# RuruX/femo

Measured on AMD Instinct MI355X. Metric: DOFs/sec assemble+adjoint-solve, 10M-DOF Poisson, 1/2/4/8 MI355X, higher is better.
Workload: dtype f64

## Files before the change

femo_amd/_lib.py:

```python
from __future__ import annotations

import ctypes as C
import os
from typing import Optional

_HERE = os.path.dirname(os.path.abspath(__file__))
LIB_PATH = os.environ.get("FEMO_LIB") or os.path.join(_HERE, "csrc", "libfemo_hip.so")

c_i64 = C.c_int64
c_i32p = C.POINTER(C.c_int32)
c_i64p = C.POINTER(C.c_int64)
c_f64p = C.POINTER(C.c_double)
H = C.c_void_p

ABI_VERSION = 10
MESH_INFO_COUNT = 12
MESH_INFO_KEYS = ("tdim", "n_vert", "n_rows", "n_cell", "nnz", "sell_entries", "max_rowlen",
                  "max_valence", "n_slices", "visit_entries", "regular_slices", "short_slices")

PDE_POISSON = 0
PDE_NL_POISSON = 1
PDE_MASS = 2
PDE_EB_BEAM = 3
J_L2_TRACKING = 0
# ... 89 lines not shown
    "femo_ctx_newton_flag_info": (C.c_int, [H, c_i64p, C.c_int]),
    "femo_mesh_create": (C.c_int, [H, C.c_int, c_i64, c_i64, C.c_void_p, c_i64, C.c_void_p, C.POINTER(H)]),
    "femo_mesh_destroy": (C.c_int, [H]),
    "femo_mesh_info": (C.c_int, [H, c_i64p]),
    "femo_mesh_set_boundary_facets": (C.c_int, [H, C.c_void_p]),
    "femo_pc_plan_host": (C.c_int, [C.c_int, C.c_int64, C.c_void_p, C.c_void_p, C.c_void_p, C.c_int64, C.POINTER(C.c_int32),
                          C.c_void_p, C.POINTER(C.c_int64), C.c_void_p, C.c_void_p, C.c_void_p, C.c_void_p, C.c_void_p]),
    "femo_emu_group_create": (C.c_int, [C.c_int, C.POINTER(H)]),
    "femo_emu_group_destroy": (C.c_int, [H]),
    "femo_comm_emulate": (C.c_int, [H, H, C.c_int]),
    "femo_comm_model": (C.c_int, [H, C.c_int, C.c_int]),
    "femo_comm_stats": (C.c_int, [H, C.POINTER(C.c_int64), C.c_int]),
    "femo_mesh_pcg_info": (C.c_int, [H, C.POINTER(C.c_int64), C.c_int]),
    "femo_mesh_head_info": (C.c_int, [H, C.POINTER(C.c_int64), C.c_int]),
    "femo_mesh_tail_info": (C.c_int, [H, C.POINTER(C.c_int64), C.c_int]),
    "femo_shell_create": (C.c_int, [H, c_i64, C.c_void_p, c_i64, C.c_void_p, c_i64, C.c_void_p, C.c_void_p, C.c_void_p, C.c_void_p, C.POINTER(H)]),
    "femo_shell_destroy": (C.c_int, [H]),
    "femo_shell_pc_create": (C.c_int, [H, C.c_int, c_i64, C.c_int, C.c_void_p] + [C.c_void_p] * 11),
    "femo_shell_pc_coarse": (C.c_int, [H, C.c_int, C.c_void_p, c_i64] + [C.c_void_p] * 6),
    "femo_shell_pc_coarse_matrix": (C.c_int, [H, H, C.c_void_p, C.c_int, C.c_void_p, C.POINTER(c_i64)]),
    "femo_shell_pc_hermite": (C.c_int, [H] + [C.c_void_p] * 11),
    "femo_shell_pc_info": (C.c_int, [H, C.POINTER(C.c_int32)]),
    "femo_shell_pc_block_items": (C.c_int, [H, C.c_int64] + [C.c_void_p] * 4),
    "femo_shell_pc_weights": (C.c_int, [H, C.c_double, C.c_double]),
    "femo_shell_pc_apply": (C.c_int, [H, H, C.c_void_p, H, H]),
    "femo_shell_pnorm_stress": (C.c_int, [H, C.c_double, C.c_double, H, H, C.c_double, C.c_double, C.c_double, C.c_double,
                                          C.POINTER(C.c_double), C.c_int, H, H]),
    "femo_shell_vm_rhs": (C.c_int, [H, C.c_double, C.c_double, H, H, C.c_double, H, H]),
    "femo_shell_p1_mass": (C.c_int, [H, H, H]),
    "femo_shell_ndof": (c_i64, [H]),
# ... 105 lines not shown
    "femo_elast_pc_setup": (C.c_int, [H, C.c_double]),
    "femo_elast_pc_info": (C.c_int, [H, c_i64p]),
    "femo_elast_pc_export_level": (C.c_int, [H, C.c_int, C.c_void_p]),
    "femo_elast_pc_apply": (C.c_int, [H, H, H]),
    "femo_elast_bench_spmv": (C.c_int, [H, H, H, C.c_int, c_f64p]),
    "femo_filter_create": (C.c_int, [H, C.c_int, c_i64, C.c_void_p, C.c_double, C.POINTER(H)]),
    "femo_filter_destroy": (C.c_int, [H]),
    "femo_filter_nnz": (C.c_int, [H, c_i64p]),
    "femo_filter_apply": (C.c_int, [H, C.c_int, H, H]),
    "femo_filter_export_csr": (C.c_int, [H, C.c_int, C.c_void_p, C.c_void_p, C.c_void_p]),
}


OPTIONAL = frozenset({"femo_mesh_pcg_info", "femo_mesh_head_info", "femo_mat_identity_solve_flag", "femo_vec_axpy_if",
                      "femo_newton_rhs_linear_if", "femo_ctx_newton_flag_info", "femo_mesh_tail_info",
                      "femo_dRdf_cell_apply_T_add_to_host", "femo_vec_get_host_promised", "femo_host_forget"})


class FemoError(RuntimeError):
    pass


_lib: Optional[C.CDLL] = None


def load() -> C.CDLL:
    global _lib
    if _lib is not None:
        return _lib
    if not os.path.exists(LIB_PATH):
        raise FemoError(
# ... 27 lines not shown
```

femo_amd/csrc/api.hip:

```cpp
#include <algorithm>

#include <atomic>

#include "femo_internal.h"

std::atomic<long long> femo_host_sync_count{0};

void femo_mat_touch(femo_mat* A) {
  static std::atomic<uint64_t> next{0};
  if (A) A->gen = ++next;
}

namespace {

__global__ void k_fill(int64_t n, double v, double* __restrict__ x) {
  for (int64_t i = (int64_t)blockIdx.x * blockDim.x + threadIdx.x; i < n; i += (int64_t)gridDim.x * blockDim.x) x[i] = v;
}

__global__ void k_axpy(int64_t n, double a, const double* __restrict__ x, double* __restrict__ y,
                       const int32_t* __restrict__ run_if, int32_t* __restrict__ count) {
  if (run_if != nullptr) {
    const bool leave = *run_if == 0;
    if (blockIdx.x == 0 && threadIdx.x == 0) atomicAdd(count + (leave ? 0 : 1), 1);
    if (leave) return;
// ... 523 lines not shown
  A->mesh = m;
  const int64_t nd = std::max<int64_t>(m->n_slices * FEMO_WAVE, 1);
  FEMO_HIP_CHECK(hipMalloc(&A->d_diag, nd * sizeof(double)));
  FEMO_HIP_CHECK(hipMalloc(&A->d_vals, std::max<int64_t>(m->sell_entries, 1) * sizeof(double) + 64));
  FEMO_HIP_CHECK(hipMemsetAsync(A->d_diag, 0, nd * sizeof(double), m->ctx->stream));
  FEMO_HIP_CHECK(hipMemsetAsync(A->d_vals, 0, std::max<int64_t>(m->sell_entries, 1) * sizeof(double), m->ctx->stream));
  *out = A;
  return 0;
}

int femo_mat_destroy(femo_mat* A) {
  if (!A) return 0;
  hipStreamSynchronize(A->mesh->ctx->stream);
  hipFree(A->d_diag); hipFree(A->d_vals); hipFree(A->d_valsT); hipFree(A->d_valsS); hipFree(A->d_s);
  hipFree(A->d_pcmask); hipFree(A->d_idrows);
  delete A;
  return 0;
}

static int note_pinned_vertices(femo_mat* A, int pde, const double* params, const femo_bc* bc) {
  femo_mesh* m = A->mesh;
  if (bc != nullptr && bc->n > 0) {
    if (A->idrows_uid != bc->uid) {
      const int64_t nb = std::max<int64_t>(m->n_vert, 1) + 64;
      if (!A->d_idrows) FEMO_HIP_CHECK(hipMalloc(&A->d_idrows, nb));
      FEMO_HIP_CHECK(hipMemcpyAsync(A->d_idrows, bc->d_mask, nb, hipMemcpyDeviceToDevice, m->ctx->stream));
      A->idrows_uid = bc->uid;
    }
    A->has_idrows = true;
  } else {
// ... 216 lines not shown
  if (m->n_rows == 0) return 0;
  int64_t* d_rp = nullptr; int32_t* d_col = nullptr; double* d_val = nullptr;
  FEMO_HIP_CHECK(hipMalloc(&d_rp, rp.size() * sizeof(int64_t)));
  FEMO_HIP_CHECK(hipMalloc(&d_col, m->nnz * sizeof(int32_t)));
  FEMO_HIP_CHECK(hipMalloc(&d_val, m->nnz * sizeof(double)));
  FEMO_HIP_CHECK(hipMemcpyAsync(d_rp, rp.data(), rp.size() * sizeof(int64_t), hipMemcpyHostToDevice, st));
  hipLaunchKernelGGL(k_export_rows, dim3((unsigned)((m->n_rows + 255) / 256)), dim3(256), 0, st, m->n_rows, m->d_mptr, m->d_cols, m->d_rowlen, m->d_rowreal, A->d_diag, A->d_vals, d_rp, d_col, d_val);
  FEMO_HIP_CHECK(hipGetLastError());
  FEMO_HIP_CHECK(hipMemcpyAsync(col, d_col, m->nnz * sizeof(int32_t), hipMemcpyDeviceToHost, st));
  FEMO_HIP_CHECK(hipMemcpyAsync(val, d_val, m->nnz * sizeof(double), hipMemcpyDeviceToHost, st));
  FEMO_HIP_CHECK(hipStreamSynchronize(st));
  hipFree(d_rp); hipFree(d_col); hipFree(d_val);
  return 0;
}

int femo_mat_diagonal(const femo_mat* A, femo_vec* d) {
  FEMO_REQUIRE(A && d, "null argument");
  FEMO_REQUIRE(d->n >= A->mesh->n_rows, "vector too small");
  femo_vec_touch(d);
  FEMO_HIP_CHECK(hipMemcpyAsync(d->d, A->d_diag, A->mesh->n_rows * sizeof(double), hipMemcpyDeviceToDevice, A->mesh->ctx->stream));
  return 0;
}

int femo_functional_value(femo_mesh* m, int kind, const double* params, const femo_vec* u,
                          const femo_vec* f, const femo_vec* u_d, double* value) {
  FEMO_REQUIRE(m && u && f && u_d && value, "null argument");
  FEMO_REQUIRE(u->n >= m->n_vert && u_d->n >= m->n_vert && f->n >= m->n_cell, "vector size mismatch in functional");
  if (m->n_nbr > 0) FEMO_TRY(femo_halo_exchange(m, const_cast<femo_vec*>(u)));
  const uint64_t key[4] = {u->uid, u->gen, u_d->uid, u_d->gen};
  return femo_launch_functional_value(m, kind, params, u->d, f->d, u_d->d, value, key);
// ... 142 lines not shown
```

femo_amd/csrc/femo_internal.h:

```cpp
#pragma once

#include <hip/hip_runtime.h>
#include <rccl/rccl.h>

#include <cstdint>
#include <cstdlib>
#include <cstdio>
#include <cstring>
#include <string>
#include <vector>

#include "femo_hip.h"
#include "femo_hip_test.h"

void femo_set_error(const char* fmt, ...);

#include <atomic>
extern std::atomic<long long> femo_host_sync_count;
inline hipError_t femo_counted_stream_sync(hipStream_t s) { femo_host_sync_count.fetch_add(1, std::memory_order_relaxed); return hipStreamSynchronize(s); }
inline hipError_t femo_counted_event_sync(hipEvent_t e) { femo_host_sync_count.fetch_add(1, std::memory_order_relaxed); return hipEventSynchronize(e); }
inline hipError_t femo_counted_device_sync() { femo_host_sync_count.fetch_add(1, std::memory_order_relaxed); return hipDeviceSynchronize(); }
#define hipStreamSynchronize(s) femo_counted_stream_sync(s)
#define hipEventSynchronize(e) femo_counted_event_sync(e)
#define hipDeviceSynchronize() femo_counted_device_sync()
// ... 303 lines not shown
  double* d_dense = nullptr;
  uint64_t* d_rowmask = nullptr;
  uint64_t uid = 0;
};

struct femo_mat {
  femo_mesh* mesh = nullptr;
  double* d_diag = nullptr;
  double* d_vals = nullptr;
  double* d_valsT = nullptr;
  bool valsT_valid = false;
  double* d_valsS = nullptr;
  double* d_s = nullptr;
  bool scaled_valid = false, scaled_transposed = false;
  bool s_valid = false;
  uint8_t* d_idrows = nullptr;
  bool has_idrows = false;
  uint64_t idrows_uid = 0;
  bool bpx_ok = false;
  uint8_t* d_pcmask = nullptr;
  bool pc_has_mask = false;
  uint64_t pc_key = 0;
  uint64_t gen = 0;
};
void femo_mat_touch(femo_mat* A);

#if defined(__HIPCC__)
__device__ __forceinline__ double femo_wave_sum(double v) {
#pragma unroll
  for (int off = 32; off > 0; off >>= 1) v += __shfl_down(v, off, 64);
// ... 83 lines not shown
  double* partials = nullptr;
  const double* dvec = nullptr;
  const int32_t* done = nullptr;
  const int32_t* slices = nullptr;
  int64_t n_slices = 0;
  hipStream_t stream = nullptr;
  bool ghost = false;
};
int femo_launch_spmv(const femo_mat* A, const double* x, double* y, const FemoSpmv& d);
int femo_halo_spmv(const femo_mat* A, double* x, double* y, const FemoSpmv& d, int* g_int, int* g_bnd, bool inflight = false);
int femo_halo_raw(femo_mesh* m, double* x, hipStream_t st);
int femo_spmv_transposed_scatter(const femo_mat* A, const double* vals, bool unit, const double* x, double* y, const int32_t* done);
inline bool femo_transpose_is_local(const femo_mesh* m) { return m->n_nbr == 0; }
int femo_mat_ensure_s(femo_mat* A);
int femo_mat_ensure_scaled(femo_mat* A, bool transpose);
int femo_launch_newton_rhs_linear(const femo_mat* K, const double* x, const double* u, const double* load,
                                  const uint8_t* bcmask, const double* bcval, double* y, int64_t slice0 = 0, int64_t n_range = -1,
                                  const int32_t* run_if = nullptr, int32_t* count = nullptr);
int femo_poisson_load_vector(femo_mesh* m, const femo_vec* f, const double** load);
int femo_poisson_load_stream_begin(femo_mesh* m, const femo_vec* f, int* n_ranges);
int femo_poisson_load_stream_range(femo_mesh* m, const femo_vec* f, int k, int64_t* slice0, int64_t* n_slices);
int femo_launch_impose_bc(femo_mesh* m, const double* u, const uint8_t* bcmask, const double* bcval, const double** ubc,
                          const int32_t* run_if = nullptr);
inline bool femo_residual_is_pipelined(const femo_mesh* m) {
  const int nbr = (m->max_rowlen + 1) & ~1;
  return nbr <= (m->tdim == 3 ? 16 : 8);
}
int femo_spmv_grid(const femo_mesh* m);
int femo_halo_exchange_on(femo_mesh* m, femo_vec* x, hipStream_t st);
int femo_mesh_classify_slices(femo_mesh* m);
// ... 73 lines not shown
```

femo_amd/csrc/solver.hip:

```cpp
#include <algorithm>
#include <climits>
#include <cmath>
#include <cstdlib>

#include "femo_internal.h"

namespace {

constexpr int S_GAMMA = 0, S_DELTA = 2, S_TOL2 = 3;
constexpr int P_DELTA = 0, P_GAMMA = 1;

__global__ __launch_bounds__(FEMO_BLOCK) void k_cg_init(int64_t n, const double* __restrict__ b, const double* __restrict__ q,
                                                        const double* __restrict__ s, double* __restrict__ r,
                                                        double* __restrict__ p, double* __restrict__ xh,
                                                        double* __restrict__ partials, const uint8_t* __restrict__ idrow) {
  __shared__ double lds[FEMO_BLOCK / 64];
  double s0 = 0.0, s1 = 0.0;
  for (int64_t i = (int64_t)blockIdx.x * FEMO_BLOCK + threadIdx.x; i < n; i += (int64_t)gridDim.x * FEMO_BLOCK) {
    const double si = s[i], bi = si * b[i];
    const double ri = q ? si * (b[i] - q[i]) : bi;
    if (idrow != nullptr && idrow[i]) {
      r[i] = 0.0; p[i] = 0.0; xh[i] = ri;
      continue;
    }
// ... 595 lines not shown
}

static int fill_info(femo_ctx* ctx, hipEvent_t end, femo_solve_info* info, int iters, int conv, double rr) {
  float ms = 0.f;
  FEMO_HIP_CHECK(hipEventElapsedTime(&ms, ctx->ev0, end));
  info->iterations = iters;
  info->converged = conv;
  info->residual_norm = std::sqrt(rr);
  info->solve_ms = ms;
  return 0;
}

static int finish_solve(femo_mat* A, const double* xh, femo_vec* x, bool zero_guess, femo_solve_info* info, int iters,
                        int conv, double rr) {
  FEMO_TRY(unscale_x(A, xh, x, zero_guess));
  return fill_info(A->mesh->ctx, A->mesh->ctx->ev1, info, iters, conv, rr);
}

struct SpmvSamples {
  static constexpr int N = 4;
  femo_ctx* ctx;
  int from;
  int n = 0;
  bool on = false;
  SpmvSamples(femo_ctx* c, int first) : ctx(c), from(first) {}
  int begin(int it) {
    on = it >= from && it < from + N;
    if (on) FEMO_HIP_CHECK(hipEventRecord(ctx->ev_pool[2 * n], ctx->stream));
    return 0;
  }
// ... 148 lines not shown
  V.x = w.xh; V.r = w.r; V.p = p0; V.q = nullptr; V.n = n; V.cur = 0; V.gv = gv; V.atol2 = 0.0;
  V.nb_q[0] = V.nb_q[1] = 0; V.Pq[0] = V.Pq[1] = nullptr;
  FEMO_TRY(femo_pc_merged_apply(m, mask, A->pc_key, V, S, ctx->d_flags, &stop));
  FEMO_HIP_CHECK(hipGetLastError());
  const bool spec_x = n > 0 && opts->zero_guess;
  if (spec_x) hipLaunchKernelGGL(k_unscale_done, dim3(2048), dim3(256), 0, st, n, 0, A->d_s, w.xh, x->d, ctx->d_flags);
  FEMO_TRY(read_back(ctx, ctx->ev1));
  const double rho0 = ctx->h_scal[MS_RR], bb = ctx->h_scal[MS_BB], gamma0 = ctx->h_scal[MS_GAMMA];
  info->rhs_norm = std::sqrt(bb);
  const int max_it = opts->max_it > 0 ? opts->max_it : 10000;
  info->spmv_ms = 0.0; info->spmv_samples = 0;
  info->pc_rhs_norm = std::sqrt(gamma0 * (rho0 > 0.0 ? bb / rho0 : 1.0));
  if (h_flags[0]) {
    info->pc_residual_norm = std::sqrt(gamma0);
    if (!spec_x && n > 0) FEMO_TRY(unscale_x(A, w.xh, x, opts->zero_guess));
    return fill_info(ctx, ctx->ev1, info, 0, (h_flags[2] || !(rho0 == rho0)) ? -1 : 1, rho0);
  }
  FEMO_TRY(femo_mat_ensure_scaled(A, false));

  SpmvSamples spmv(ctx, 2);
  const int batch = opts->check_every > 0 ? std::min(opts->check_every, 8) : 8;
  int predicted = 0;
  {
    const double tolg = ctx->h_scal[MS_TOLG];
    if (m->pcg_rate > 0.0 && gamma0 > 0.0 && tolg > 0.0 && gamma0 > tolg) {
      const double need = std::log(gamma0 / tolg);
      predicted = (int)std::ceil(need / m->pcg_rate) + 1;
      predicted = std::max(1, std::min(predicted, 4 * std::max(m->pcg_last_iters, 8)));
    } else if (m->pcg_rate <= 0.0) {
      const int last2 = std::min(m->pcg_last_iters, m->pcg_prev_iters);
// ... 43 lines not shown
  info->loop_allreduces = (int32_t)(ctx->n_allreduce - ar0);
  const hipEvent_t end = h_flags[0] ? ctx->ev_pool[POLL_EV] : ctx->ev1;
  if (!h_flags[0]) {
    if (R) flush(false, true);
    else if (n > 0) hipLaunchKernelGGL(k_unscale, dim3(2048), dim3(256), 0, st, n, opts->zero_guess ? 0 : 1, A->d_s, w.xh, x->d);
    FEMO_TRY(read_back(ctx, ctx->ev1));
  }
  const int iters = h_flags[1];
  const int conv = h_flags[0] ? (h_flags[2] ? -1 : 1) : 0;
  if (conv == 1 && iters > 0) { m->pcg_prev_iters = m->pcg_last_iters; m->pcg_last_iters = iters; }
  if (conv == 1 && iters >= 4) {
    const double g_end = ctx->h_scal[MS_GAMMA + (iters & 1)];
    if (g_end > 0.0 && gamma0 > g_end) m->pcg_rate = std::log(gamma0 / g_end) / iters;
  }
  FEMO_TRY(spmv.report(info));
  info->pc_residual_norm = std::sqrt(ctx->h_scal[MS_GAMMA + (iters & 1)]);
  return fill_info(ctx, end, info, iters, conv, ctx->h_scal[MS_RR]);
}

static int solve_pcg_bpx(femo_mat* A, int transpose, const femo_vec* b, femo_vec* x,
                         const femo_solver_opts* opts, femo_solve_info* info) {
  femo_mesh* m = A->mesh;
  femo_ctx* ctx = m->ctx;
  const int64_t n = m->n_rows;
  FEMO_REQUIRE(A->bpx_ok, "the BPX preconditioner needs an operator assembled from a Poisson-type form");
  FEMO_REQUIRE(!transpose, "the BPX preconditioner is for symmetric operators");
  hipStream_t st = ctx->stream;
  if (!(ctx->comm != nullptr && ctx->nranks == 1 && femo_env_flag("FEMO_FORCE_MULTI")) && femo_pc_merged_ok(m))
    return solve_pcg_bpx_merged(A, b, x, opts, info);
  FEMO_HIP_CHECK(hipEventRecord(ctx->ev0, st));
// ... 352 lines not shown
```

femo_amd/csrc/spmv.hip:

```cpp
#include <algorithm>
#include <climits>
#include <cmath>
#include <cstdlib>

#include "femo_internal.h"

namespace {

typedef double femo_v2d __attribute__((ext_vector_type(2)));
typedef int femo_v2i __attribute__((ext_vector_type(2)));

__device__ __forceinline__ double2 nt_load2(const double2* p) {
  const femo_v2d v = __builtin_nontemporal_load(reinterpret_cast<const femo_v2d*>(p));
  return make_double2(v.x, v.y);
}
__device__ __forceinline__ int2 nt_load2(const int2* p) {
  const femo_v2i v = __builtin_nontemporal_load(reinterpret_cast<const femo_v2i*>(p));
  return make_int2(v.x, v.y);
}
template <bool NT> __device__ __forceinline__ double2 mat_load2(const double2* p) {
  if constexpr (NT) return nt_load2(p);
  else { const femo_v2d v = *reinterpret_cast<const femo_v2d*>(p); return make_double2(v.x, v.y); }
}
template <bool NT> __device__ __forceinline__ int mat_load(const int* p) {
// ... 178 lines not shown
__device__ __forceinline__ double row_sum_gh(int npair, const double2* __restrict__ v2, const int2* __restrict__ c2,
                                             const double* __restrict__ x, const double* __restrict__ gbase, int n_own, double acc) {
  while (npair > 4) {
    acc = row_pairs_gh<4, NT>(v2, c2, x, gbase, n_own, acc);
    v2 += 4 * 64; c2 += 4 * 64; npair -= 4;
  }
  switch (npair) {
    case 4: return row_pairs_gh<4, NT>(v2, c2, x, gbase, n_own, acc);
    case 3: return row_pairs_gh<3, NT>(v2, c2, x, gbase, n_own, acc);
    case 2: return row_pairs_gh<2, NT>(v2, c2, x, gbase, n_own, acc);
    case 1: return row_pairs_gh<1, NT>(v2, c2, x, gbase, n_own, acc);
    default: return acc;
  }
}

template <int DOT, bool UNIT, bool NT = true, bool GH = false>
__global__ __launch_bounds__(FEMO_BLOCK) void k_spmv_sell(
    int64_t n_rows, int64_t n_slices, const int64_t* __restrict__ mptr,
    const int32_t* __restrict__ cols, const int16_t* __restrict__ cols16, const int32_t* __restrict__ sdelta, int sdelta_stride,
    const double* __restrict__ vals, const double* __restrict__ diag, const double* __restrict__ x,
    double* __restrict__ y, double* __restrict__ partials, const int32_t* __restrict__ done,
    const int32_t* __restrict__ slice_list, int64_t n_list, const double* __restrict__ dvec, SpmvGhost gh = SpmvGhost{}) {
  if (done != nullptr && *done) return;
  bool waited = false;
  __shared__ double lds[FEMO_BLOCK / 64];
  const int lane = threadIdx.x & 63;
  const int wave = __builtin_amdgcn_readfirstlane(threadIdx.x >> 6);
  const int xcd = blockIdx.x & 7;
  const int64_t blk_in_xcd = blockIdx.x >> 3;
  const int64_t waves_per_xcd = (int64_t)(gridDim.x >> 3) * (FEMO_BLOCK / 64);
  const int64_t n_walk = slice_list ? n_list : n_slices;
  const int64_t s_lo = n_walk * xcd / 8, s_hi = n_walk * (xcd + 1) / 8;
  double dot = 0.0, dot2 = 0.0, dot3 = 0.0;
  for (int64_t si = s_lo + blk_in_xcd * (FEMO_BLOCK / 64) + wave; si < s_hi; si += waves_per_xcd) {
    const int32_t entry = slice_list ? slice_list[si] : (int32_t)si;
    const bool bnd = GH && entry < 0;
    const int64_t slice = GH ? (int64_t)(entry & 0x7FFFFFFF) : (slice_list ? (int64_t)entry : si);
    const int64_t base = mptr[slice];
    const int npair = (int)((mptr[slice + 1] - base) >> 7);
    const int64_t row = (slice << 6) + lane;
    if (GH && bnd && !waited) { spmv_halo_wait_wave(gh, lane); waited = true; }
    const double xr = x[row < n_rows ? row : 0];
    double acc = UNIT ? xr : diag[row] * xr;
    const double2* __restrict__ v2 = reinterpret_cast<const double2*>(vals + base) + lane;
    const int32_t* __restrict__ dl = sdelta + slice * sdelta_stride;
    if (GH && bnd) {
      const int2* __restrict__ c2 = reinterpret_cast<const int2*>(cols + base) + lane;
      acc = row_sum_gh<NT>(npair, v2, c2, x, gh.ghost - gh.n_own, (int)gh.n_own, acc);
    } else if (dl[0] != INT32_MIN) {
      acc = row_sum_regular<NT>(npair, v2, dl, x + row, acc);
    } else if (dl[1] == 1) {
      const int* __restrict__ c16 = reinterpret_cast<const int*>(cols16) + (base >> 1) + lane;
      acc = row_sum_short<NT>(npair, v2, c16, x + row, acc);
    } else {
      const int2* __restrict__ c2 = reinterpret_cast<const int2*>(cols + base) + lane;
      acc = row_sum<NT>(npair, v2, c2, x, acc);
    }
    if (row < n_rows) {
      y[row] = acc;
      if (DOT == 4) {
// ... 123 lines not shown
    tperm[e] = t;
  }
}

__global__ void k_gather(int64_t n, const int32_t* __restrict__ perm, const double* __restrict__ in,
                         double* __restrict__ out) {
  for (int64_t i = (int64_t)blockIdx.x * blockDim.x + threadIdx.x; i < n; i += (int64_t)gridDim.x * blockDim.x)
    out[i] = in[perm[i]];
}

__global__ void k_invsqrt_diag(int64_t n, const double* __restrict__ diag, double* __restrict__ s) {
  for (int64_t i = (int64_t)blockIdx.x * blockDim.x + threadIdx.x; i < n; i += (int64_t)gridDim.x * blockDim.x)
    s[i] = 1.0 / sqrt(diag[i]);
}

__global__ __launch_bounds__(FEMO_BLOCK) void k_scale_sell(int64_t n_slices, const int64_t* __restrict__ mptr,
                                                           const int32_t* __restrict__ cols, const int32_t* __restrict__ sdelta,
                                                           int sdelta_stride, const double* __restrict__ vals,
                                                           const double* __restrict__ s, int64_t n_vert, double* __restrict__ out) {
  const int lane = threadIdx.x & 63;
  const int64_t nw = (int64_t)gridDim.x * (FEMO_BLOCK / 64);
  for (int64_t slice = (int64_t)blockIdx.x * (FEMO_BLOCK / 64) + (threadIdx.x >> 6); slice < n_slices; slice += nw) {
    const int64_t base = mptr[slice];
    const int wm = (int)((mptr[slice + 1] - base) >> 6);
    const int64_t row = (slice << 6) + lane;
    const double si = s[row < n_vert ? row : 0];
    const int32_t* dl = sdelta + slice * sdelta_stride;
    const bool regular = dl[0] != INT32_MIN;
    for (int k = 0; k < wm; k += 2) {
      const int64_t idx = base + (int64_t)(k >> 1) * 128 + lane * 2;
      const double2 v = *reinterpret_cast<const double2*>(vals + idx);
      int64_t c0, c1;
      if (regular) { c0 = row + dl[k]; c1 = row + dl[k + 1]; }
      else { const int2 cc = *reinterpret_cast<const int2*>(cols + idx); c0 = cc.x; c1 = cc.y; }
      double2 o;
      o.x = si * v.x * s[c0];
      o.y = si * v.y * s[c1];
      *reinterpret_cast<double2*>(out + idx) = o;
    }
  }
}

__global__ void k_pack(int64_t n, const int32_t* __restrict__ idx, const double* __restrict__ x, double* __restrict__ buf) {
  for (int64_t i = (int64_t)blockIdx.x * blockDim.x + threadIdx.x; i < n; i += (int64_t)gridDim.x * blockDim.x) buf[i] = x[idx[i]];
}

}

int femo_spmv_grid(const femo_mesh* m) {
  int64_t g = (m->n_slices + 3) / 4;
  const int64_t cap = (int64_t)m->ctx->n_cu * 4;
  if (g > cap) g = cap;
  if (g > FEMO_MAX_PARTIALS) g = FEMO_MAX_PARTIALS;
// ... 8 lines not shown

static bool matrix_streams(const femo_mesh* m) {
  return (int64_t)m->sell_entries * (int64_t)sizeof(double) > FEMO_LLC_MATRIX_BYTES;
}

int femo_launch_spmv(const femo_mat* A, const double* x, double* y, const FemoSpmv& d) {
  const femo_mesh* m = A->mesh;
  FEMO_REQUIRE(d.dots == FEMO_DOTS_NONE || d.partials != nullptr, "product with dots: no partials to write them to");
  FEMO_REQUIRE(d.dots <= FEMO_DOTS_DAX || d.unit, "product with dots %d: unit-diagonal operators only", (int)d.dots);
  FEMO_REQUIRE(d.dots != FEMO_DOTS_TRIPLE || d.dvec != nullptr, "product with the merged triple: no dvec");
  FEMO_REQUIRE(!d.ghost || (d.dots == FEMO_DOTS_TRIPLE && d.unit && d.slices), "ghost-aware product: merged-loop variant only");
  const int64_t n_walk = d.slices ? d.n_slices : m->n_slices;
  if (n_walk == 0 && d.dots == FEMO_DOTS_NONE) return 0;
  const int g = d.slices ? subset_grid(m, n_walk) : femo_spmv_grid(m);
  hipStream_t st = d.stream ? d.stream : m->ctx->stream;
#define FEMO_SPMV_ARGS m->n_rows, m->n_slices, m->d_mptr, m->d_cols, m->d_cols16, m->d_sdelta, m->sdelta_stride, d.vals, A->d_diag, x, y, d.partials, d.done, d.slices, d.n_slices, d.dvec
  const bool nt = matrix_streams(m);
#define FEMO_SPMV_LAUNCH(DOT, UNIT)                                                                                     \
  do {                                                                                                                  \
    if (nt) hipLaunchKernelGGL((k_spmv_sell<DOT, UNIT, true>), dim3(g), dim3(FEMO_BLOCK), 0, st, FEMO_SPMV_ARGS);        \
    else hipLaunchKernelGGL((k_spmv_sell<DOT, UNIT, false>), dim3(g), dim3(FEMO_BLOCK), 0, st, FEMO_SPMV_ARGS);          \
  } while (0)
  switch (d.dots) {
    case FEMO_DOTS_NONE:
      if (d.unit) FEMO_SPMV_LAUNCH(FEMO_DOTS_NONE, true);
      else FEMO_SPMV_LAUNCH(FEMO_DOTS_NONE, false);
      break;
    case FEMO_DOTS_DAX:
      if (d.unit) FEMO_SPMV_LAUNCH(FEMO_DOTS_DAX, true);
      else FEMO_SPMV_LAUNCH(FEMO_DOTS_DAX, false);
      break;
    case FEMO_DOTS_DAX_XX: FEMO_SPMV_LAUNCH(FEMO_DOTS_DAX_XX, true); break;
    case FEMO_DOTS_DAX_AXAX: FEMO_SPMV_LAUNCH(FEMO_DOTS_DAX_AXAX, true); break;
    case FEMO_DOTS_TRIPLE:
      if (d.ghost) {
// ... 253 lines not shown
int femo_mat_ensure_s(femo_mat* A) {
  femo_mesh* m = A->mesh;
  femo_ctx* ctx = m->ctx;
  if (A->s_valid) return 0;
  const int64_t nd = std::max<int64_t>(m->n_vert, m->n_slices * FEMO_WAVE) + 2;
  if (!A->d_s) FEMO_HIP_CHECK(hipMalloc(&A->d_s, nd * sizeof(double)));
  if (m->n_rows > 0) {
    hipLaunchKernelGGL(k_invsqrt_diag, dim3(2048), dim3(256), 0, ctx->stream, m->n_rows, A->d_diag, A->d_s);
    FEMO_HIP_CHECK(hipGetLastError());
  }
  if (m->n_nbr > 0) FEMO_TRY(femo_halo_raw(m, A->d_s, ctx->stream));
  A->s_valid = true;
  return 0;
}

int femo_mat_ensure_scaled(femo_mat* A, bool transpose) {
  femo_mesh* m = A->mesh;
  femo_ctx* ctx = m->ctx;
  if (A->scaled_valid && A->scaled_transposed == transpose) return 0;
  const double* src = A->d_vals;
  if (transpose) {
    FEMO_TRY(femo_mat_ensure_transpose(A));
    src = A->d_valsT;
  }
  FEMO_TRY(femo_mat_ensure_s(A));
  if (!A->d_valsS) FEMO_HIP_CHECK(hipMalloc(&A->d_valsS, std::max<int64_t>(m->sell_entries, 1) * sizeof(double) + 64));
  if (m->n_slices > 0) {
    hipLaunchKernelGGL(k_scale_sell, dim3(2048), dim3(FEMO_BLOCK), 0, ctx->stream, m->n_slices, m->d_mptr, m->d_cols, m->d_sdelta, m->sdelta_stride, src, A->d_s, m->n_vert, A->d_valsS);
    FEMO_HIP_CHECK(hipGetLastError());
  }
  A->scaled_valid = true;
  A->scaled_transposed = transpose;
  return 0;
}

extern "C" int femo_bench_spmv(const femo_mat* A, const femo_vec* x, femo_vec* y, int reps, double* ms_per_launch) {
  FEMO_REQUIRE(A && x && y && ms_per_launch && reps > 0, "bad argument");
  femo_ctx* ctx = A->mesh->ctx;
  FEMO_REQUIRE(x->n >= A->mesh->n_vert && y->n >= A->mesh->n_rows, "vector size mismatch");
  femo_vec_touch(y);
  FEMO_TRY(femo_mat_ensure_scaled(const_cast<femo_mat*>(A), false));
  const FemoSpmv Ap = {.vals = A->d_valsS, .unit = true, .dots = FEMO_DOTS_DAX, .partials = ctx->d_partials + 3 * FEMO_MAX_PARTIALS};
  for (int i = 0; i < 3; ++i) FEMO_TRY(femo_launch_spmv(A, x->d, y->d, Ap));
// ... 1 lines not shown
  for (int i = 0; i < reps; ++i) FEMO_TRY(femo_launch_spmv(A, x->d, y->d, Ap));
  FEMO_HIP_CHECK(hipEventRecord(ctx->ev1, ctx->stream));
  FEMO_HIP_CHECK(hipEventSynchronize(ctx->ev1));
  float ms = 0.f;
  FEMO_HIP_CHECK(hipEventElapsedTime(&ms, ctx->ev0, ctx->ev1));
  *ms_per_launch = (double)ms / reps;
  return 0;
}

extern "C" int femo_mat_prescale(femo_mat* A) {
  FEMO_REQUIRE(A != nullptr, "null argument");
  FEMO_TRY(femo_mat_ensure_scaled(A, false));
  if (!A->bpx_ok) return 0;
  return femo_pc_weights_early(A->mesh, A->d_s, A->pc_has_mask ? A->d_pcmask : nullptr, femo_pc_weights_key(A));
}
```

femo_amd/engine.py:

```python
from __future__ import annotations

import contextlib
import ctypes as C
import threading
from typing import Dict, List, Optional, Sequence

import numpy as np

from . import _lib
from ._lib import FemoError, H, SolveInfo, SolverOpts, check


PC_KINDS = {"jacobi": 0, "bpx": 1}


def _f64(a) -> np.ndarray:
    return np.ascontiguousarray(a, dtype=np.float64)


def _i32(a) -> np.ndarray:
    return np.ascontiguousarray(a, dtype=np.int32)


def _ptr(a: Optional[np.ndarray]):
# ... 645 lines not shown
        info = SolveInfo()
        check(self.lib.femo_solve_cg(self.handle, int(transpose), b.handle, x.handle, C.byref(opts), C.byref(info)))
        return info

    def pc_apply(self, r: Vec, z: Vec) -> Vec:
        check(self.lib.femo_mat_pc_apply(self.handle, r.handle, z.handle))
        return z

    def solve_bicgstab(self, b: Vec, x: Vec, transpose: bool = False, rtol: float = 1e-12, atol: float = 0.0,
                       max_it: int = 100000, zero_guess: bool = True, check_every: int = 32) -> SolveInfo:
        opts = SolverOpts(rtol, atol, max_it, int(zero_guess), check_every, 0, 0.0)
        info = SolveInfo()
        check(self.lib.femo_solve_bicgstab(self.handle, int(transpose), b.handle, x.handle, C.byref(opts), C.byref(info)))
        return info

    def bench_spmv(self, x: Vec, y: Vec, reps: int = 50) -> float:
        ms = C.c_double(0.0)
        check(self.lib.femo_bench_spmv(self.handle, x.handle, y.handle, reps, C.byref(ms)))
        return ms.value

    def __del__(self):
        try:
            h, self.handle = getattr(self, "handle", None), None
            if h and getattr(self.mesh, "handle", None) and getattr(self.mesh.ctx, "handle", None):
                self.lib.femo_mat_destroy(h)
        except Exception:
            pass


def _params(params) -> Optional[np.ndarray]:
# ... 137 lines not shown
```

Measured before the change: 206.1 million.

## Pack zero-valued pairs out of regular SELL slices for the scaled SpMV

While scaling the matrix, the scale kernel also builds a compacted copy of the regular slices. Column pairs whose scaled values are zero across the whole wave are dropped, and per-slice pair counts and compacted delta tables are recorded. Single-rank CG SpMV then uses this compact layout to read fewer values. The compact path is disabled when less than an eighth of pairs would be removed. It costs an extra value array, extra writes during scaling and a host-visible counter, and it adds CSR import and debug entry points.

```diff
diff --git a/femo_amd/_lib.py b/femo_amd/_lib.py
--- a/femo_amd/_lib.py
+++ b/femo_amd/_lib.py
@@ -127,6 +127,9 @@
     "femo_mesh_pcg_info": (C.c_int, [H, C.POINTER(C.c_int64), C.c_int]),
     "femo_mesh_head_info": (C.c_int, [H, C.POINTER(C.c_int64), C.c_int]),
     "femo_mesh_tail_info": (C.c_int, [H, C.POINTER(C.c_int64), C.c_int]),
+    "femo_mat_compact_info": (C.c_int, [H, C.POINTER(C.c_int64), C.c_int]),
+    "femo_mat_spmv_scaled": (C.c_int, [H, C.c_int, H, H, c_f64p, C.POINTER(C.c_int)]),
+    "femo_mat_import_csr": (C.c_int, [H, C.c_void_p]),
     "femo_shell_create": (C.c_int, [H, c_i64, C.c_void_p, c_i64, C.c_void_p, c_i64, C.c_void_p, C.c_void_p, C.c_void_p, C.c_void_p, C.POINTER(H)]),
     "femo_shell_destroy": (C.c_int, [H]),
     "femo_shell_pc_create": (C.c_int, [H, C.c_int, c_i64, C.c_int, C.c_void_p] + [C.c_void_p] * 11),
@@ -262,7 +265,8 @@
 
 OPTIONAL = frozenset({"femo_mesh_pcg_info", "femo_mesh_head_info", "femo_mat_identity_solve_flag", "femo_vec_axpy_if",
                       "femo_newton_rhs_linear_if", "femo_ctx_newton_flag_info", "femo_mesh_tail_info",
-                      "femo_dRdf_cell_apply_T_add_to_host", "femo_vec_get_host_promised", "femo_host_forget"})
+                      "femo_dRdf_cell_apply_T_add_to_host", "femo_vec_get_host_promised", "femo_host_forget",
+                      "femo_mat_compact_info", "femo_mat_spmv_scaled", "femo_mat_import_csr"})
 
 
 class FemoError(RuntimeError):
diff --git a/femo_amd/csrc/api.hip b/femo_amd/csrc/api.hip
--- a/femo_amd/csrc/api.hip
+++ b/femo_amd/csrc/api.hip
@@ -561,6 +561,7 @@
   hipStreamSynchronize(A->mesh->ctx->stream);
   hipFree(A->d_diag); hipFree(A->d_vals); hipFree(A->d_valsT); hipFree(A->d_valsS); hipFree(A->d_s);
   hipFree(A->d_pcmask); hipFree(A->d_idrows);
+  femo_mat_compact_free(A);
   delete A;
   return 0;
 }
@@ -807,6 +808,47 @@
   return 0;
 }
 
+__global__ void k_import_rows(int64_t n_rows, const int64_t* __restrict__ mptr, const int32_t* __restrict__ cols,
+                              const int32_t* __restrict__ rowlen, const uint32_t* __restrict__ rowreal, double* __restrict__ diag,
+                              double* __restrict__ vals, const int64_t* __restrict__ rowptr, const double* __restrict__ ival) {
+  const int64_t row = (int64_t)blockIdx.x * blockDim.x + threadIdx.x;
+  if (row >= n_rows) return;
+  const int64_t base = mptr[row >> 6];
+  const int lane = (int)(row & 63);
+  const int len = rowlen[row];
+  int64_t o = rowptr[row];
+  bool placed = false;
+  const uint32_t real = rowreal[row];
+  for (int k = 0; k < len; ++k) {
+    if (k < 32 && !((real >> k) & 1u)) continue;
+    const int64_t e = femo_sell_index(base, k, lane);
+    if (!placed && cols[e] > row) { diag[row] = ival[o]; ++o; placed = true; }
+    vals[e] = ival[o]; ++o;
+  }
+  if (!placed) diag[row] = ival[o];
+}
+
+int femo_mat_import_csr(femo_mat* A, const double* val) {
+  FEMO_REQUIRE(A && val, "null argument");
+  const femo_mesh* m = A->mesh;
+  hipStream_t st = m->ctx->stream;
+  A->valsT_valid = false; A->scaled_valid = false; A->s_valid = false; femo_mat_touch(A);
+  if (m->n_rows == 0) return 0;
+  std::vector<int64_t> rp;
+  FEMO_TRY(pattern_rowptr(m, rp));
+  int64_t* d_rp = nullptr; double* d_val = nullptr;
+  FEMO_HIP_CHECK(hipMalloc(&d_rp, rp.size() * sizeof(int64_t)));
+  FEMO_HIP_CHECK(hipMalloc(&d_val, m->nnz * sizeof(double)));
+  FEMO_HIP_CHECK(hipMemcpyAsync(d_rp, rp.data(), rp.size() * sizeof(int64_t), hipMemcpyHostToDevice, st));
+  FEMO_HIP_CHECK(hipMemcpyAsync(d_val, val, m->nnz * sizeof(double), hipMemcpyHostToDevice, st));
+  FEMO_HIP_CHECK(hipMemsetAsync(A->d_vals, 0, std::max<int64_t>(m->sell_entries, 1) * sizeof(double), st));
+  hipLaunchKernelGGL(k_import_rows, dim3((unsigned)((m->n_rows + 255) / 256)), dim3(256), 0, st, m->n_rows, m->d_mptr, m->d_cols, m->d_rowlen, m->d_rowreal, A->d_diag, A->d_vals, d_rp, d_val);
+  FEMO_HIP_CHECK(hipGetLastError());
+  FEMO_HIP_CHECK(hipStreamSynchronize(st));
+  hipFree(d_rp); hipFree(d_val);
+  return 0;
+}
+
 int femo_mat_diagonal(const femo_mat* A, femo_vec* d) {
   FEMO_REQUIRE(A && d, "null argument");
   FEMO_REQUIRE(d->n >= A->mesh->n_rows, "vector too small");
diff --git a/femo_amd/csrc/femo_internal.h b/femo_amd/csrc/femo_internal.h
--- a/femo_amd/csrc/femo_internal.h
+++ b/femo_amd/csrc/femo_internal.h
@@ -341,6 +341,16 @@
   double* d_s = nullptr;
   bool scaled_valid = false, scaled_transposed = false;
   bool s_valid = false;
+  double* d_valsC = nullptr;
+  int32_t* d_cdelta = nullptr;
+  int32_t* d_cpairs = nullptr;
+  unsigned long long* d_ccount = nullptr;
+  unsigned long long* h_ccount = nullptr;
+  bool compact_valid = false;
+  bool compact_off = false;
+  bool compact_pending = false;
+  mutable int64_t products_compact = 0, products_full = 0;
+  int64_t compact_live = 0, compact_full = 0, compact_slices = 0;
   uint8_t* d_idrows = nullptr;
   bool has_idrows = false;
   uint64_t idrows_uid = 0;
@@ -454,6 +464,8 @@
 inline bool femo_transpose_is_local(const femo_mesh* m) { return m->n_nbr == 0; }
 int femo_mat_ensure_s(femo_mat* A);
 int femo_mat_ensure_scaled(femo_mat* A, bool transpose);
+void femo_mat_compact_settle(femo_mat* A);
+void femo_mat_compact_free(femo_mat* A);
 int femo_launch_newton_rhs_linear(const femo_mat* K, const double* x, const double* u, const double* load,
                                   const uint8_t* bcmask, const double* bcval, double* y, int64_t slice0 = 0, int64_t n_range = -1,
                                   const int32_t* run_if = nullptr, int32_t* count = nullptr);
diff --git a/femo_amd/csrc/solver.hip b/femo_amd/csrc/solver.hip
--- a/femo_amd/csrc/solver.hip
+++ b/femo_amd/csrc/solver.hip
@@ -633,6 +633,7 @@
 static int finish_solve(femo_mat* A, const double* xh, femo_vec* x, bool zero_guess, femo_solve_info* info, int iters,
                         int conv, double rr) {
   FEMO_TRY(unscale_x(A, xh, x, zero_guess));
+  femo_mat_compact_settle(A);
   return fill_info(A->mesh->ctx, A->mesh->ctx->ev1, info, iters, conv, rr);
 }
 
@@ -811,6 +812,7 @@
   if (h_flags[0]) {
     info->pc_residual_norm = std::sqrt(gamma0);
     if (!spec_x && n > 0) FEMO_TRY(unscale_x(A, w.xh, x, opts->zero_guess));
+    femo_mat_compact_settle(A);
     return fill_info(ctx, ctx->ev1, info, 0, (h_flags[2] || !(rho0 == rho0)) ? -1 : 1, rho0);
   }
   FEMO_TRY(femo_mat_ensure_scaled(A, false));
@@ -884,6 +886,7 @@
     if (g_end > 0.0 && gamma0 > g_end) m->pcg_rate = std::log(gamma0 / g_end) / iters;
   }
   FEMO_TRY(spmv.report(info));
+  femo_mat_compact_settle(A);
   info->pc_residual_norm = std::sqrt(ctx->h_scal[MS_GAMMA + (iters & 1)]);
   return fill_info(ctx, end, info, iters, conv, ctx->h_scal[MS_RR]);
 }
diff --git a/femo_amd/csrc/spmv.hip b/femo_amd/csrc/spmv.hip
--- a/femo_amd/csrc/spmv.hip
+++ b/femo_amd/csrc/spmv.hip
@@ -216,13 +216,14 @@
   }
 }
 
-template <int DOT, bool UNIT, bool NT = true, bool GH = false>
+template <int DOT, bool UNIT, bool NT = true, bool GH = false, bool CP = false>
 __global__ __launch_bounds__(FEMO_BLOCK) void k_spmv_sell(
     int64_t n_rows, int64_t n_slices, const int64_t* __restrict__ mptr,
     const int32_t* __restrict__ cols, const int16_t* __restrict__ cols16, const int32_t* __restrict__ sdelta, int sdelta_stride,
     const double* __restrict__ vals, const double* __restrict__ diag, const double* __restrict__ x,
     double* __restrict__ y, double* __restrict__ partials, const int32_t* __restrict__ done,
-    const int32_t* __restrict__ slice_list, int64_t n_list, const double* __restrict__ dvec, SpmvGhost gh = SpmvGhost{}) {
+    const int32_t* __restrict__ slice_list, int64_t n_list, const double* __restrict__ dvec,
+    const int32_t* __restrict__ cdelta, const int32_t* __restrict__ cpairs, SpmvGhost gh = SpmvGhost{}) {
   if (done != nullptr && *done) return;
   bool waited = false;
   __shared__ double lds[FEMO_BLOCK / 64];
@@ -239,13 +240,13 @@
     const bool bnd = GH && entry < 0;
     const int64_t slice = GH ? (int64_t)(entry & 0x7FFFFFFF) : (slice_list ? (int64_t)entry : si);
     const int64_t base = mptr[slice];
-    const int npair = (int)((mptr[slice + 1] - base) >> 7);
+    const int npair = CP ? cpairs[slice] : (int)((mptr[slice + 1] - base) >> 7);
     const int64_t row = (slice << 6) + lane;
     if (GH && bnd && !waited) { spmv_halo_wait_wave(gh, lane); waited = true; }
     const double xr = x[row < n_rows ? row : 0];
     double acc = UNIT ? xr : diag[row] * xr;
     const double2* __restrict__ v2 = reinterpret_cast<const double2*>(vals + base) + lane;
-    const int32_t* __restrict__ dl = sdelta + slice * sdelta_stride;
+    const int32_t* __restrict__ dl = (CP ? cdelta : sdelta) + slice * sdelta_stride;
     if (GH && bnd) {
       const int2* __restrict__ c2 = reinterpret_cast<const int2*>(cols + base) + lane;
       acc = row_sum_gh<NT>(npair, v2, c2, x, gh.ghost - gh.n_own, (int)gh.n_own, acc);
@@ -399,12 +400,17 @@
     s[i] = 1.0 / sqrt(diag[i]);
 }
 
+template <bool PACK>
 __global__ __launch_bounds__(FEMO_BLOCK) void k_scale_sell(int64_t n_slices, const int64_t* __restrict__ mptr,
                                                            const int32_t* __restrict__ cols, const int32_t* __restrict__ sdelta,
                                                            int sdelta_stride, const double* __restrict__ vals,
-                                                           const double* __restrict__ s, int64_t n_vert, double* __restrict__ out) {
+                                                           const double* __restrict__ s, int64_t n_vert, double* __restrict__ out,
+                                                           double* __restrict__ outC, int32_t* __restrict__ cdelta,
+                                                           int32_t* __restrict__ cpairs, unsigned long long* __restrict__ count,
+                                                           unsigned long long* __restrict__ hcount) {
   const int lane = threadIdx.x & 63;
   const int64_t nw = (int64_t)gridDim.x * (FEMO_BLOCK / 64);
+  unsigned long long n_live = 0, n_full = 0, n_reg = 0;
   for (int64_t slice = (int64_t)blockIdx.x * (FEMO_BLOCK / 64) + (threadIdx.x >> 6); slice < n_slices; slice += nw) {
     const int64_t base = mptr[slice];
     const int wm = (int)((mptr[slice + 1] - base) >> 6);
@@ -412,6 +418,10 @@
     const double si = s[row < n_vert ? row : 0];
     const int32_t* dl = sdelta + slice * sdelta_stride;
     const bool regular = dl[0] != INT32_MIN;
+    int32_t* cd = PACK ? cdelta + slice * sdelta_stride : nullptr;
+    int p = 0;
+    double2 pend;
+    pend.x = 0.0; pend.y = 0.0;
     for (int k = 0; k < wm; k += 2) {
       const int64_t idx = base + (int64_t)(k >> 1) * 128 + lane * 2;
       const double2 v = *reinterpret_cast<const double2*>(vals + idx);
@@ -422,6 +432,54 @@
       o.x = si * v.x * s[c0];
       o.y = si * v.y * s[c1];
       *reinterpret_cast<double2*>(out + idx) = o;
+      if (PACK) {
+        if (!regular) {
+          *reinterpret_cast<double2*>(outC + idx) = o;
+        } else {
+          if (__ballot(!(o.x == 0.0)) != 0ull) {
+            if (p & 1) { pend.y = o.x; *reinterpret_cast<double2*>(outC + base + (int64_t)(p >> 1) * 128 + lane * 2) = pend; }
+            else pend.x = o.x;
+            if (lane == 0) cd[p] = dl[k];
+            ++p;
+          }
+          if (__ballot(!(o.y == 0.0)) != 0ull) {
+            if (p & 1) { pend.y = o.y; *reinterpret_cast<double2*>(outC + base + (int64_t)(p >> 1) * 128 + lane * 2) = pend; }
+            else pend.x = o.y;
+            if (lane == 0) cd[p] = dl[k + 1];
+            ++p;
+          }
+        }
+      }
+    }
+    if (PACK) {
+      if (regular) {
+        if (p & 1) {
+          pend.y = 0.0;
+          *reinterpret_cast<double2*>(outC + base + (int64_t)(p >> 1) * 128 + lane * 2) = pend;
+          if (lane == 0) cd[p] = 0;
+          ++p;
+        }
+        for (int i = p + lane; i < sdelta_stride; i += 64) cd[i] = 0;
+        ++n_reg;
+      } else {
+        for (int i = lane; i < sdelta_stride; i += 64) cd[i] = dl[i];
+        p = wm;
+      }
+      if (lane == 0) cpairs[slice] = p >> 1;
+      n_live += (unsigned long long)(p >> 1);
+      n_full += (unsigned long long)(wm >> 1);
+    }
+  }
+  if (PACK && lane == 0) {
+    if (n_live) atomicAdd(count, n_live);
+    if (n_full) atomicAdd(count + 1, n_full);
+    if (n_reg) atomicAdd(count + 2, n_reg);
+    __threadfence();
+    if (atomicAdd(count + 3, 1ull) == (unsigned long long)gridDim.x * (FEMO_BLOCK / 64) - 1ull) {
+      __threadfence();
+      for (int i = 0; i < 3; ++i)
+        __hip_atomic_store(hcount + i, atomicExch(count + i, 0ull), __ATOMIC_RELAXED, __HIP_MEMORY_SCOPE_SYSTEM);
+      atomicExch(count + 3, 0ull);
     }
   }
 }
@@ -460,11 +518,19 @@
   if (n_walk == 0 && d.dots == FEMO_DOTS_NONE) return 0;
   const int g = d.slices ? subset_grid(m, n_walk) : femo_spmv_grid(m);
   hipStream_t st = d.stream ? d.stream : m->ctx->stream;
-#define FEMO_SPMV_ARGS m->n_rows, m->n_slices, m->d_mptr, m->d_cols, m->d_cols16, m->d_sdelta, m->sdelta_stride, d.vals, A->d_diag, x, y, d.partials, d.done, d.slices, d.n_slices, d.dvec
+  const bool compact = d.vals == A->d_valsS && d.unit && A->scaled_valid && A->compact_valid && d.slices == nullptr && !d.ghost;
+  const double* vals = compact ? A->d_valsC : d.vals;
+  const int32_t* cdelta = compact ? A->d_cdelta : nullptr;
+  const int32_t* cpairs = compact ? A->d_cpairs : nullptr;
+  if (d.vals == A->d_valsS) ++(compact ? A->products_compact : A->products_full);
+#define FEMO_SPMV_ARGS m->n_rows, m->n_slices, m->d_mptr, m->d_cols, m->d_cols16, m->d_sdelta, m->sdelta_stride, vals, A->d_diag, x, y, d.partials, d.done, d.slices, d.n_slices, d.dvec, cdelta, cpairs
   const bool nt = matrix_streams(m);
 #define FEMO_SPMV_LAUNCH(DOT, UNIT)                                                                                     \
   do {                                                                                                                  \
-    if (nt) hipLaunchKernelGGL((k_spmv_sell<DOT, UNIT, true>), dim3(g), dim3(FEMO_BLOCK), 0, st, FEMO_SPMV_ARGS);        \
+    if (compact) {                                                                                                      \
+      if (nt) hipLaunchKernelGGL((k_spmv_sell<DOT, true, true, false, true>), dim3(g), dim3(FEMO_BLOCK), 0, st, FEMO_SPMV_ARGS);   \
+      else hipLaunchKernelGGL((k_spmv_sell<DOT, true, false, false, true>), dim3(g), dim3(FEMO_BLOCK), 0, st, FEMO_SPMV_ARGS);     \
+    } else if (nt) hipLaunchKernelGGL((k_spmv_sell<DOT, UNIT, true>), dim3(g), dim3(FEMO_BLOCK), 0, st, FEMO_SPMV_ARGS);  \
     else hipLaunchKernelGGL((k_spmv_sell<DOT, UNIT, false>), dim3(g), dim3(FEMO_BLOCK), 0, st, FEMO_SPMV_ARGS);          \
   } while (0)
   switch (d.dots) {
@@ -748,6 +814,50 @@
   return 0;
 }
 
+static bool compact_wanted(const femo_mat* A) {
+  const femo_mesh* m = A->mesh;
+  if (A->compact_off || m->ctx->nranks > 1 || m->n_nbr > 0 || m->n_slices == 0) return false;
+  const char* e = getenv("FEMO_SPMV_COMPACT");
+  if (e != nullptr && e[0] == '0' && e[1] == 0) return false;
+  return 2 * m->n_regular >= m->n_slices;
+}
+
+static bool compact_alloc(femo_mat* A) {
+  const femo_mesh* m = A->mesh;
+  if (A->d_valsC != nullptr) return true;
+  const size_t nv = (size_t)std::max<int64_t>(m->sell_entries, 1) * sizeof(double) + 64;
+  const size_t nd = (size_t)m->n_slices * (size_t)m->sdelta_stride * sizeof(int32_t);
+  const bool ok = hipMalloc(&A->d_valsC, nv) == hipSuccess && hipMalloc(&A->d_cdelta, nd) == hipSuccess &&
+                  hipMalloc(&A->d_cpairs, (size_t)m->n_slices * sizeof(int32_t)) == hipSuccess &&
+                  hipMalloc(&A->d_ccount, 4 * sizeof(unsigned long long)) == hipSuccess &&
+                  hipHostMalloc(&A->h_ccount, 3 * sizeof(unsigned long long)) == hipSuccess &&
+                  hipMemsetAsync(A->d_ccount, 0, 4 * sizeof(unsigned long long), m->ctx->stream) == hipSuccess;
+  if (!ok) {
+    (void)hipGetLastError();
+    femo_mat_compact_free(A);
+    A->compact_off = true;
+  }
+  return ok;
+}
+
+void femo_mat_compact_free(femo_mat* A) {
+  hipFree(A->d_valsC); hipFree(A->d_cdelta); hipFree(A->d_cpairs); hipFree(A->d_ccount);
+  if (A->h_ccount) hipHostFree(A->h_ccount);
+  A->d_valsC = nullptr; A->d_cdelta = nullptr; A->d_cpairs = nullptr; A->d_ccount = nullptr; A->h_ccount = nullptr;
+  A->compact_valid = false; A->compact_pending = false;
+}
+
+void femo_mat_compact_settle(femo_mat* A) {
+  if (!A->compact_pending) return;
+  A->compact_pending = false;
+  const unsigned long long live = A->h_ccount[0], full = A->h_ccount[1];
+  A->compact_live = (int64_t)live; A->compact_full = (int64_t)full; A->compact_slices = (int64_t)A->h_ccount[2];
+  if ((full - live) * 8ull < full) {
+    femo_mat_compact_free(A);
+    A->compact_off = true;
+  }
+}
+
 int femo_mat_ensure_scaled(femo_mat* A, bool transpose) {
   femo_mesh* m = A->mesh;
   femo_ctx* ctx = m->ctx;
@@ -759,8 +869,18 @@
   }
   FEMO_TRY(femo_mat_ensure_s(A));
   if (!A->d_valsS) FEMO_HIP_CHECK(hipMalloc(&A->d_valsS, std::max<int64_t>(m->sell_entries, 1) * sizeof(double) + 64));
+  A->compact_valid = false;
+  const bool pack = compact_wanted(A) && compact_alloc(A);
   if (m->n_slices > 0) {
-    hipLaunchKernelGGL(k_scale_sell, dim3(2048), dim3(FEMO_BLOCK), 0, ctx->stream, m->n_slices, m->d_mptr, m->d_cols, m->d_sdelta, m->sdelta_stride, src, A->d_s, m->n_vert, A->d_valsS);
+#define FEMO_SCALE_ARGS m->n_slices, m->d_mptr, m->d_cols, m->d_sdelta, m->sdelta_stride, src, A->d_s, m->n_vert, A->d_valsS
+    if (pack) {
+      hipLaunchKernelGGL((k_scale_sell<true>), dim3(2048), dim3(FEMO_BLOCK), 0, ctx->stream, FEMO_SCALE_ARGS, A->d_valsC, A->d_cdelta, A->d_cpairs, A->d_ccount, A->h_ccount);
+      A->compact_pending = true;
+      A->compact_valid = true;
+    } else {
+      hipLaunchKernelGGL((k_scale_sell<false>), dim3(2048), dim3(FEMO_BLOCK), 0, ctx->stream, FEMO_SCALE_ARGS, (double*)nullptr, (int32_t*)nullptr, (int32_t*)nullptr, (unsigned long long*)nullptr, (unsigned long long*)nullptr);
+    }
+#undef FEMO_SCALE_ARGS
     FEMO_HIP_CHECK(hipGetLastError());
   }
   A->scaled_valid = true;
@@ -792,3 +912,36 @@
   if (!A->bpx_ok) return 0;
   return femo_pc_weights_early(A->mesh, A->d_s, A->pc_has_mask ? A->d_pcmask : nullptr, femo_pc_weights_key(A));
 }
+
+extern "C" int femo_mat_compact_info(femo_mat* A, int64_t* out, int count) {
+  FEMO_REQUIRE(A && out, "null argument");
+  FEMO_HIP_CHECK(hipStreamSynchronize(A->mesh->ctx->stream));
+  if (A->compact_pending) {
+    A->compact_live = (int64_t)A->h_ccount[0]; A->compact_full = (int64_t)A->h_ccount[1]; A->compact_slices = (int64_t)A->h_ccount[2];
+  }
+  const int64_t v[6] = {(A->scaled_valid && A->compact_valid) ? 1 : 0, A->compact_slices, A->compact_live, A->compact_full,
+                        A->products_compact, A->products_full};
+  for (int i = 0; i < 6 && i < count; ++i) out[i] = v[i];
+  return 0;
+}
+
+extern "C" int femo_mat_spmv_scaled(femo_mat* A, int dots, const femo_vec* x, femo_vec* y, double* partials, int* nblocks) {
+  FEMO_REQUIRE(A && x && y, "null argument");
+  FEMO_REQUIRE(dots >= FEMO_DOTS_NONE && dots <= FEMO_DOTS_DAX_AXAX, "dots %d: 0 .. 3", dots);
+  FEMO_REQUIRE(dots == FEMO_DOTS_NONE || (partials && nblocks), "product with dots: no room for the partials");
+  femo_mesh* m = A->mesh;
+  femo_ctx* ctx = m->ctx;
+  FEMO_REQUIRE(m->n_nbr == 0, "one rank only");
+  FEMO_REQUIRE(x->n >= m->n_vert && y->n >= m->n_rows && x->d != y->d, "vector size mismatch");
+  FEMO_TRY(femo_vec_await(x));
+  femo_vec_touch(y);
+  FEMO_TRY(femo_mat_ensure_scaled(A, false));
+  double* P = ctx->d_partials + 3 * FEMO_MAX_PARTIALS;
+  FEMO_TRY(femo_launch_spmv(A, x->d, y->d, {.vals = A->d_valsS, .unit = true, .dots = (FemoSpmvDots)dots, .partials = dots ? P : nullptr}));
+  const int g = femo_spmv_grid(m);
+  for (int k = 0; k < femo_spmv_dot_slots((FemoSpmvDots)dots); ++k)
+    FEMO_HIP_CHECK(hipMemcpyAsync(partials + (size_t)k * g, P + (size_t)k * FEMO_MAX_PARTIALS, (size_t)g * sizeof(double), hipMemcpyDeviceToHost, ctx->stream));
+  FEMO_HIP_CHECK(hipStreamSynchronize(ctx->stream));
+  if (nblocks) *nblocks = g;
+  return 0;
+}
diff --git a/femo_amd/engine.py b/femo_amd/engine.py
--- a/femo_amd/engine.py
+++ b/femo_amd/engine.py
@@ -683,6 +683,24 @@
         check(self.lib.femo_solve_bicgstab(self.handle, int(transpose), b.handle, x.handle, C.byref(opts), C.byref(info)))
         return info
 
+    def compact_info(self) -> Dict[str, int]:
+        out = (C.c_int64 * 6)()
+        check(self.lib.femo_mat_compact_info(self.handle, out, 6))
+        return dict(zip(("valid", "slices", "live_pairs", "full_pairs", "products_compact", "products_full"), (int(v) for v in out)))
+
+    def spmv_scaled(self, dots: int, x: Vec, y: Vec):
+        part = np.zeros(2 * 2048, np.float64)
+        nb = C.c_int(0)
+        check(self.lib.femo_mat_spmv_scaled(self.handle, int(dots), x.handle, y.handle, part.ctypes.data_as(C.POINTER(C.c_double)), C.byref(nb)))
+        sums = {0: 0, 1: 1, 2: 2, 3: 2}[int(dots)]
+        return part[:sums * nb.value].reshape(sums, nb.value).copy()
+
+    def import_csr(self, val) -> "Mat":
+        val = _f64(val)
+        assert val.size == self.mesh.info["nnz"]
+        check(self.lib.femo_mat_import_csr(self.handle, _ptr(val)))
+        return self
+
     def bench_spmv(self, x: Vec, y: Vec, reps: int = 50) -> float:
         ms = C.c_double(0.0)
         check(self.lib.femo_bench_spmv(self.handle, x.handle, y.handle, reps, C.byref(ms)))
```

New measurement: 239.5 million (median of 6 runs). 1.16x the previous value.
